# noiseinspacechannel/NIS-SAR-AMTIGMTI-Video

Measured on AMD Instinct MI355X. Metric: focused SAR frames/sec (CSA focus, complex64), higher is better.
Workload: dtype c64 (phase arguments f64)

## Files before the change

### nis-sar-amtigmti-video_amd/csrc/api_csa.hip

```cpp
#include "api_ctx.h"
#include "csa_kernels.h"
#include "general.h"

#include <cmath>
#include <cstdlib>
#include <string>
#include <vector>

using namespace sarx;

struct sarx_plan {
    sarx_ctx* ctx = nullptr;
    int n_az = 0, n_rg = 0;
    unsigned flags = 0;
    sarx_radar_params p{};
    int az_s = 0;
    int az_w = 32;
    int az_w_alone = 0;
    int az_impl = 1;
    int az_wpb = 4;
    int look = 0;
    float* look_slot = nullptr;
    float* look_part = nullptr;
    const float2* ati_s1 = nullptr; const float* ati_thr = nullptr; float ati_frac = 0.f; double ati_cal = 0.0;
    float *ati_phase = nullptr, *ati_m1 = nullptr, *ati_dm = nullptr; int ati_keep_image = 0;
    double2* ati_part = nullptr; int ati_nparts = 0;
    int ati_w = 32;
    float* max_slot = nullptr;
    bool az_nt = false;
    int slab_tiles = 0;
    double2 *c1 = nullptr, *c2 = nullptr, *c3 = nullptr;
    float2* buf_b = nullptr;
    float2* buf_a = nullptr;
    float2 *h_in = nullptr, *h_out = nullptr;
    static constexpr int PIPE = 2;
    float2 *pipe_in[PIPE] = {}, *pipe_out[PIPE] = {};
    int pipe_dl[PIPE] = {-1, -1};
    void* pipe_host[PIPE] = {};
    int pipe_next = 0;
    uint64_t bytes = 0;
    int mark_start = -1, mark_stop = -1;
    unsigned long long* stamp = nullptr;
    GeneralCsa* gen = nullptr;
// ... 186 lines not shown
                                                        "products need whole waves (sarx_ati_dpca_dev otherwise)", p->n_az, p->n_rg, tpt);
    p->ati_w = w;
    const int tiles = (p->az_s == p->n_az ? 1 : p->n_az / p->az_s) * (p->n_rg / w);
    const int waves = tpt / 64;
    if (!p->ati_part) {
        hipError_t e = hipMalloc(&p->ati_part, ((size_t)tiles * waves + 128) * sizeof(double2));
        if (e != hipSuccess) return fail(c, SARX_ERR_NOMEM, "hipMalloc ATI partial sums: %s", hipGetErrorString(e));
        p->bytes += (size_t)tiles * waves * sizeof(double2);
    }
    p->ati_nparts = tiles * waves;
    p->ati_s1 = (const float2*)d_slc1; p->ati_thr = d_max; p->ati_frac = mask_frac; p->ati_cal = cal_phase;
    p->ati_phase = d_ati_phase_masked; p->ati_m1 = d_slc1_mag; p->ati_dm = d_dpca_mag; p->ati_keep_image = keep_image != 0;
    return SARX_OK;
}

int sarx_csa_plan_bytes(const sarx_plan* p, uint64_t* out) {
    if (!p || !out) return fail(p ? p->ctx : nullptr, SARX_ERR_INVALID, "NULL argument");
    *out = p->bytes;
    return SARX_OK;
}

int sarx_csa_axes(const sarx_plan* p, double* range_axis, double* cross_range_axis) {
    if (!p) return fail(nullptr, SARX_ERR_INVALID, "plan is NULL");
    const double dt = 1.0 / p->p.sample_rate_hz;
    if (range_axis)
        for (int j = 0; j < p->n_rg; ++j) range_axis[j] = C_LIGHT * (p->p.t_start_fast_s + (double)j * dt) / 2.0;
    if (cross_range_axis) {
        double mean = 0.0;
        for (int i = 0; i < p->n_az; ++i) mean += (double)i / p->p.prf_hz;
        mean /= (double)p->n_az;
// ... 46 lines not shown
    a.ati_part = p->ati_part; a.ati_keep_image = p->ati_keep_image;
}
static int ati_finish(sarx_plan* p) {
    if (!p->ati_s1) return SARX_OK;
    sarx_ctx* c = p->ctx;
    HIPCHK(c, launch_ati_finish_sums(p->ati_part, p->ati_nparts, p->ati_thr, p->ati_part + p->ati_nparts, c->ati_out3_(), c->stream));
    return SARX_OK;
}
struct AzLast { int epi, w; };
static AzLast az_last(const sarx_plan* p, bool inv, int w_plain, AzArgs& a) {
    const bool look = inv && p->look_slot;
    if (look) { a.look_part = p->look_part; a.look = p->look; }
    const bool ati = inv && p->ati_s1;
    if (inv && !ati) a.max_out = reinterpret_cast<unsigned*>(p->max_slot);
    if (ati) ati_args(p, a);
    return {inv ? (ati ? AZ_EPI_SCALE_ATI : look ? AZ_EPI_SCALE_LOOK : AZ_EPI_SCALE) : AZ_EPI_PHI1, ati ? p->ati_w : look ? p->az_w : w_plain};
}
static int az_step(sarx_plan* p, bool inv, bool step_b, int S, const void* in, void* out, int q0, int nq) {
    sarx_ctx* c = p->ctx;
    const int n = p->n_az, RA = n / S;
    AzArgs a = az_args(p, in, out);
    a.q0 = q0;
    const bool alone = !(c->range_cus > 0 && c->range_cus < c->cus);
    const int w_plain = (alone && p->az_w_alone) ? p->az_w_alone : p->az_w;
    const auto wave = [&](int r, int epi) { return p->az_impl && n == 16384 && az_wave_supported(r, p->n_rg, epi, p->az_wpb); };
    if (!step_b) {
        a.tw_r = c->tw_all + RA;
        a.in_q_stride = 1; a.in_m_stride = S; a.out_q_stride = 1; a.out_m_stride = S;
        if (wave(RA, AZ_EPI_TWIDDLE)) HIPCHK(c, launch_az_wave(inv, AZ_EPI_TWIDDLE, p->az_wpb, a, nq, c->stream));
        else HIPCHK(c, launch_az_tile(RA, w_plain, inv, AZ_EPI_TWIDDLE, a, nq, c->stream));
    } else {
// ... 135 lines not shown
    if (p->flags & SARX_FUSE_RANGE) {
        RangeArgs a = range_args(p, p->buf_b, p->buf_b);
        a.stamp = p->stamp;
        HIPCHK(c, run_range(p, RG_FUSED, a));
    } else if (range_wp_supported(p->n_rg) && (c->range_impl == 0 || c->range_impl == 4)) {
        RangeArgs a = range_args(p, p->buf_b, p->buf_b);
        HIPCHK(c, launch_range_wp(RG_FFT_PHI2, a, c->cus, c->stream));
        HIPCHK(c, launch_range_wp(RG_IFFT_PHI3, a, c->cus, c->stream));
    } else {
        RangeArgs a = range_args(p, p->buf_b, p->buf_b);
        HIPCHK(c, run_range(p, RG_FFT_PHI2, a));
        HIPCHK(c, run_range(p, RG_IFFT_PHI3, a));
    }
    if (p->mark_stop >= 0) { HIPCHK(c, hipEventRecord(c->ev[p->mark_stop], c->stream)); c->ev_set[p->mark_stop] = true; }
    float2* last = rg_major ? p->buf_a : (float2*)d_image;
    if (p->az_s == p->n_az) {
        if ((rc = az_pass(p, true, p->buf_b, nullptr, last)) != SARX_OK) return rc;
    } else {
        if ((rc = az_pass(p, true, p->buf_b, p->buf_b, last)) != SARX_OK) return rc;
    }
    if ((rc = look_finish(p)) != SARX_OK) return rc;
    if ((rc = ati_finish(p)) != SARX_OK) return rc;
    if (rg_major) HIPCHK(c, launch_corner_turn(p->buf_a, (float2*)d_image, p->n_az, p->n_rg, c->stream));
    return SARX_OK;
}


int sarx_csa_focus_host_c128(sarx_plan* p, const void* phist_host, void* image_host) {
    if (!p) return fail(nullptr, SARX_ERR_INVALID, "plan is NULL");
    sarx_ctx* c = p->ctx;
    hipSetDevice(c->device);
// ... 71 lines not shown
```

### nis-sar-amtigmti-video_amd/csrc/csa_kernels.h

```cpp
#pragma once
#include <hip/hip_runtime.h>
#include <stddef.h>
#include <stdint.h>

namespace sarx {

enum RangeMode { RG_FFT = 0, RG_IFFT = 1, RG_FFT_PHI2 = 2, RG_IFFT_PHI3 = 3, RG_FUSED = 4,
                 RG_CONV = 5 };
enum AzEpilogue { AZ_EPI_NONE = 0, AZ_EPI_TWIDDLE = 1, AZ_EPI_PHI1 = 2, AZ_EPI_SCALE = 3,
                  AZ_EPI_TWCOL = 4,
                  AZ_EPI_PROCOL = 5,
                  AZ_EPI_ROWVEC = 6,
                  AZ_EPI_TWIDDLE_PADIN = 7,
                  AZ_EPI_CROPOUT = 8,
                  AZ_EPI_TWIDDLE_ROWSIN = 9,
                  AZ_EPI_SCALE_ROWSOUT = 10,
                  AZ_EPI_CROPOUT_PHI1 = 11,
                  AZ_EPI_CROPOUT_MAG = 12,
                  AZ_EPI_SCALE_LOOK = 13,
                  AZ_EPI_SCALE_ATI = 14 };

struct RangeArgs {
    const float2* in;
    float2* out;
    const float2* tw;
    const double2* c2;
    const double2* c3;
    double df;
    double dt;
    double t_start;
    double t0;
    float inv_n;
    int n_az;
    const float2* mulvec;
// ... 172 lines not shown
```

### nis-sar-amtigmti-video_amd/csrc/csa_kernels.hip

```cpp
#include <type_traits>
#include "csa_kernels.h"
#include "fft_core.hpp"
#include "phase.hpp"
#include "ati_pixel.hpp"

namespace sarx {

template <int N> struct RangeCfg {
    using PL = Plan<N>;
    static constexpr int T = PL::T;
    static constexpr int ROWS = (T >= 256) ? 1 : 256 / T;
    static constexpr int THREADS = T * ROWS;
    static constexpr int LDS_PER_ROW = LdsSize<N, 1>::value;
    static constexpr size_t LDS_BYTES = (size_t)ROWS * LDS_PER_ROW * sizeof(cf);
};

template <int N, int MODE>
__global__ __launch_bounds__(RangeCfg<N>::THREADS, (N == 4096 && MODE == RG_CONV) ? 4 : 1) void range_pass_kernel(RangeArgs a) {
    using CFG = RangeCfg<N>;
    using PL = Plan<N>;
    constexpr int P = PL::P, T = PL::T;
    extern __shared__ __attribute__((aligned(16))) char smem_raw[];
    cf* lds = reinterpret_cast<cf*>(smem_raw);

// ... 168 lines not shown
    static constexpr int TPC = PL::T;
    static constexpr int THREADS = TPC * W;
    static constexpr size_t LDS_BYTES = (PL::nstages > 1) ? (size_t)LdsSize<R, W>::value * sizeof(cf) : 0;
};

typedef float nt_v2f __attribute__((ext_vector_type(2)));
__device__ __forceinline__ cf ld_stream(const cf* p, bool nt) {
    if (nt) { const nt_v2f v = __builtin_nontemporal_load(reinterpret_cast<const nt_v2f*>(p)); return make_float2(v.x, v.y); }
    return *p;
}
__device__ __forceinline__ void st_stream(cf* p, cf x, bool nt) {
    if (nt) __builtin_nontemporal_store(nt_v2f{x.x, x.y}, reinterpret_cast<nt_v2f*>(p));
    else *p = x;
}

template <int R, int W, bool INV, int EPI>
__global__ __launch_bounds__((AzCfg<R, W>::THREADS)) void az_tile_kernel(AzArgs a) {
    using PL = Plan<R>;
    using E = Edge<R, false>;
    constexpr int P = PL::P;
    extern __shared__ __attribute__((aligned(16))) char smem_raw[];
    cf* lds = reinterpret_cast<cf*>(smem_raw);

    const int c = threadIdx.x % W;
    const int t = threadIdx.x / W;
    const int col = blockIdx.x * W + c;
    const int q = blockIdx.y + a.q0;
    const size_t in_base = (size_t)q * a.in_q_stride;
    const size_t out_base = (size_t)q * a.out_q_stride;

    cf v[P];
    constexpr int R0 = E::R_first;
#pragma unroll
    for (int b = 0; b < P / R0; ++b)
#pragma unroll
        for (int r = 0; r < R0; ++r) {
            const int mi = E::in_index(t, b, r);
            const size_t rowi = in_base + (size_t)mi * a.in_m_stride;
            cf x;
            if constexpr (EPI == AZ_EPI_TWIDDLE_PADIN) {
                x = make_float2(0.f, 0.f);
                if (rowi < (size_t)a.io_rows && col < a.io_cols) {
                    size_t srow = rowi + (size_t)a.io_shift_in;
                    if (srow >= (size_t)a.io_rows) srow -= (size_t)a.io_rows;
                    x = a.in[srow * a.io_ld + col];
                }
            } else if constexpr (EPI == AZ_EPI_TWIDDLE_ROWSIN) {
// ... 17 lines not shown
                for (int r = 0; r < R0; ++r) {
                    const size_t rowi = in_base + (size_t)E::in_index(t, b, r) * a.in_m_stride;
                    if (rowi >= (size_t)a.io_rows) continue;
                    cf& x = v[b * R0 + r];
                    if (a.hamming_inv > 0.f) {
                        size_t srow = rowi + (size_t)a.io_shift_in;
                        if (srow >= (size_t)a.io_rows) srow -= (size_t)a.io_rows;
                        const float w = fmaf(-0.46f, __builtin_amdgcn_cosf((float)srow * a.hamming_inv), 0.54f);
                        x.x *= w; x.y *= w;
                    } else {
                        x = cmul(x, a.rowvec[rowi]);
                    }
                }
        }
    }
    float ati_thr = 0.f;
    double ati_re = 0.0, ati_im = 0.0;
    if constexpr (EPI == AZ_EPI_SCALE_ATI) {
        __shared__ float s_m[AzCfg<R, W>::THREADS / 64 > 0 ? AzCfg<R, W>::THREADS / 64 : 1];
        float m = 0.f;
        for (unsigned k = threadIdx.x; k < MAX_SHARDS; k += AzCfg<R, W>::THREADS) m = fmaxf(m, a.ati_thr[32 * k]);
        for (int off = 32; off > 0; off >>= 1) m = fmaxf(m, __shfl_xor(m, off, 64));
        if ((threadIdx.x & 63) == 0) s_m[threadIdx.x >> 6] = m;
        __syncthreads();
        m = s_m[0];
        for (int k = 1; k < AzCfg<R, W>::THREADS / 64; ++k) m = fmaxf(m, s_m[k]);
        ati_thr = m * a.ati_frac;
    }
    cf s1v[EPI == AZ_EPI_SCALE_ATI ? P : 1];
    if constexpr (EPI == AZ_EPI_SCALE_ATI) {
        constexpr int RLp = E::R_last;
#pragma unroll
        for (int b = 0; b < P / RLp; ++b)
#pragma unroll
            for (int r = 0; r < RLp; ++r)
                s1v[b * RLp + r] = a.ati_s1[(out_base + (size_t)E::out_index(t, b, r) * a.out_m_stride) * a.n_rg + col];
    }
    stockham_run<R, W, INV, false, 0, false, (R == 128)>(v, t, c, lds, a.tw_r);
    constexpr int RL = E::R_last;
    float vmax = 0.f;
#pragma unroll
    for (int b = 0; b < P / RL; ++b)
#pragma unroll
        for (int r = 0; r < RL; ++r) {
            const int m = E::out_index(t, b, r);
            const size_t rowo = out_base + (size_t)m * a.out_m_stride;
            cf x = v[b * RL + r];
            if constexpr (EPI == AZ_EPI_TWIDDLE || EPI == AZ_EPI_TWIDDLE_PADIN || EPI == AZ_EPI_TWIDDLE_ROWSIN) {
#if SARX_HW_TWIDDLE
                const float rev = (float)(q * m) * a.scale;
                x = cmul(x, cis_frac(INV ? rev : -rev));
#else
                cf w = a.tw_n[(size_t)q * m];
                if (INV) w = cconj(w);
                x = cmul(x, w);
#endif
            } else if constexpr (EPI == AZ_EPI_PHI1) {
                x = cmul(x, phi1(col, a.c1[rowo], a.dt, a.t_start));
            } else if constexpr (EPI == AZ_EPI_SCALE_ATI) {
                x.x *= a.scale; x.y *= a.scale;
                const size_t o = rowo * a.n_rg + col;
                Pix px;
                ati_pixel<false>(s1v[b * RL + r], x, a.ati_cc, a.ati_cs, px);
                a.ati_phase[o] = px.m1 > ati_thr ? px.phase : 0.f;
                a.ati_m1[o] = px.m1;
                a.ati_dm[o] = px.dm;
                ati_re += px.sre; ati_im += px.sim;
                if (!a.ati_keep_image) continue;
            } else if constexpr (EPI == AZ_EPI_SCALE_LOOK) {
                x.x *= a.scale; x.y *= a.scale;
                if (a.max_out) vmax = fmaxf(vmax, hypotf(x.x, x.y));
                float pw = fmaf(x.x, x.x, x.y * x.y);
                auto dpp_add = [&](auto ctrl) {
                    pw += __int_as_float(__builtin_amdgcn_update_dpp(0, __float_as_int(pw), decltype(ctrl)::value, 0xF, 0xF, false));
                };
                if (a.look > 1) dpp_add(std::integral_constant<int, 0xB1>{});
                if (a.look > 2) dpp_add(std::integral_constant<int, 0x4E>{});
                if (a.look > 4) dpp_add(std::integral_constant<int, 0x141>{});
                if (a.look > 8) dpp_add(std::integral_constant<int, 0x140>{});
                for (int off = 16; off < a.look; off <<= 1) pw += __shfl_xor(pw, off, 64);
                if ((c & (a.look - 1)) == 0) a.look_part[rowo * (size_t)(a.n_rg / a.look) + col / a.look] = pw;
            } else if constexpr (EPI == AZ_EPI_SCALE || EPI == AZ_EPI_PROCOL) {
                if constexpr (EPI == AZ_EPI_PROCOL) {
                    if (a.valid_len && m * a.n_rg + col >= a.valid_len) continue;
                }
                x.x *= a.scale; x.y *= a.scale;
                if constexpr (EPI == AZ_EPI_SCALE) { if (a.max_out) vmax = fmaxf(vmax, hypotf(x.x, x.y)); }
            } else if constexpr (EPI == AZ_EPI_SCALE_ROWSOUT) {
                if (rowo >= (size_t)a.io_rows) continue;
                x.x *= a.scale; x.y *= a.scale;
            } else if constexpr (EPI == AZ_EPI_ROWVEC) {
                x = cmul(x, a.rowvec[rowo]);
            } else if constexpr (EPI == AZ_EPI_CROPOUT || EPI == AZ_EPI_CROPOUT_PHI1 || EPI == AZ_EPI_CROPOUT_MAG) {
                if (rowo < (size_t)a.io_rows && col < a.io_cols) {
                    x.x *= a.scale; x.y *= a.scale;
                    if (a.rowvec) x = cmul(x, a.rowvec[rowo]);
                    if constexpr (EPI == AZ_EPI_CROPOUT_PHI1) x = cmul(x, phi1(col, a.c1[rowo], a.dt, a.t_start));
                    size_t drow = rowo + (size_t)a.io_shift_out;
                    if (drow >= (size_t)a.io_rows) drow -= (size_t)a.io_rows;
                    if constexpr (EPI == AZ_EPI_CROPOUT_MAG) a.out_mag[drow * a.io_ld + col] = hypotf(x.x, x.y);
                    else a.out[drow * a.io_ld + col] = x;
                }
                continue;
            } else if constexpr (EPI == AZ_EPI_TWCOL) {
                const float rev = (float)(col * m) * a.tw_scale;
                x = cmul(x, cis_frac(INV ? rev : -rev));
            }
            st_stream(a.out + rowo * a.n_rg + col, x, a.nt);
        }
    if constexpr (EPI == AZ_EPI_SCALE_ATI) {
        for (int off = 32; off > 0; off >>= 1) { ati_re += __shfl_xor(ati_re, off, 64); ati_im += __shfl_xor(ati_im, off, 64); }
        if ((threadIdx.x & 63) == 0)
            a.ati_part[((size_t)blockIdx.y * gridDim.x + blockIdx.x) * (AzCfg<R, W>::THREADS / 64) + (threadIdx.x >> 6)] = make_double2(ati_re, ati_im);
    }
    if constexpr (EPI == AZ_EPI_SCALE || EPI == AZ_EPI_SCALE_LOOK) {
        if (a.max_out) {
            for (int off = 32; off > 0; off >>= 1) vmax = fmaxf(vmax, __shfl_xor(vmax, off, 64));
            if ((threadIdx.x & 63) == 0)
                atomicMax(a.max_out + 32u * ((blockIdx.x * 7u + blockIdx.y * 13u + (threadIdx.x >> 6)) & (MAX_SHARDS - 1u)), __float_as_uint(vmax));
        }
    }
}

template <int R, int W, bool INV, int EPI> static hipError_t launch_az_one(const AzArgs& a, int nq, hipStream_t st) {
    using CFG = AzCfg<R, W>;
    dim3 grid(a.n_rg / W, nq);
    hipLaunchKernelGGL((az_tile_kernel<R, W, INV, EPI>), grid, dim3(CFG::THREADS), CFG::LDS_BYTES, st, a);
    return hipGetLastError();
}
template <int R, int W> static hipError_t launch_az_rw(bool inv, int epi, const AzArgs& a, int nq, hipStream_t st) {
// ... 4 lines not shown
            case AZ_EPI_PHI1: return launch_az_one<R, W, false, AZ_EPI_PHI1>(a, nq, st);
            case AZ_EPI_TWCOL: return launch_az_one<R, W, false, AZ_EPI_TWCOL>(a, nq, st);
            case AZ_EPI_ROWVEC: return launch_az_one<R, W, false, AZ_EPI_ROWVEC>(a, nq, st);
            case AZ_EPI_TWIDDLE_PADIN: return launch_az_one<R, W, false, AZ_EPI_TWIDDLE_PADIN>(a, nq, st);
            case AZ_EPI_TWIDDLE_ROWSIN: return launch_az_one<R, W, false, AZ_EPI_TWIDDLE_ROWSIN>(a, nq, st);
            case AZ_EPI_CROPOUT:
                if constexpr (R >= 16 && W == 32) return launch_az_one<R, W, false, AZ_EPI_CROPOUT>(a, nq, st); else return hipErrorInvalidValue;
        }
    } else {
        switch (epi) {
            case AZ_EPI_NONE: return launch_az_one<R, W, true, AZ_EPI_NONE>(a, nq, st);
            case AZ_EPI_TWIDDLE: return launch_az_one<R, W, true, AZ_EPI_TWIDDLE>(a, nq, st);
            case AZ_EPI_SCALE: return launch_az_one<R, W, true, AZ_EPI_SCALE>(a, nq, st);
            case AZ_EPI_SCALE_LOOK: return launch_az_one<R, W, true, AZ_EPI_SCALE_LOOK>(a, nq, st);
            case AZ_EPI_SCALE_ATI: if constexpr (AzCfg<R, W>::THREADS % 64 == 0) return launch_az_one<R, W, true, AZ_EPI_SCALE_ATI>(a, nq, st); else return hipErrorInvalidValue;
            case AZ_EPI_PROCOL: return launch_az_one<R, W, true, AZ_EPI_PROCOL>(a, nq, st);
            case AZ_EPI_CROPOUT: return launch_az_one<R, W, true, AZ_EPI_CROPOUT>(a, nq, st);
            case AZ_EPI_SCALE_ROWSOUT: return launch_az_one<R, W, true, AZ_EPI_SCALE_ROWSOUT>(a, nq, st);
            case AZ_EPI_CROPOUT_PHI1: return launch_az_one<R, W, true, AZ_EPI_CROPOUT_PHI1>(a, nq, st);
            case AZ_EPI_CROPOUT_MAG: return launch_az_one<R, W, true, AZ_EPI_CROPOUT_MAG>(a, nq, st);
        }
    }
    return hipErrorInvalidValue;
}
template <int R> static hipError_t launch_az_r(int w, bool inv, int epi, const AzArgs& a, int nq, hipStream_t st) {
    switch (w) {
        case 16: return launch_az_rw<R, 16>(inv, epi, a, nq, st);
        case 32: return launch_az_rw<R, 32>(inv, epi, a, nq, st);
        case 64: return launch_az_rw<R, 64>(inv, epi, a, nq, st);
    }
// ... 76 lines not shown
```

### nis-sar-amtigmti-video_amd/sarx/_ffi.py

```python
from __future__ import annotations

import ctypes as C
import os

_HERE = os.path.dirname(os.path.abspath(__file__))
LIB_PATH = os.environ.get("SARX_LIB") or os.path.join(_HERE, "libsarx.so")

MAX_SLOT_BYTES = 32768
COMM_ID_BYTES = 128
OUT_AZ_MAJOR, OUT_RG_MAJOR, FUSE_RANGE = 0, 1, 2
PASS_AZ_FFT_PHI1, PASS_RG_FFT_PHI2, PASS_RG_IFFT_PHI3, PASS_AZ_IFFT, PASS_RG_FUSED_23 = 1, 2, 3, 4, 23
PASS_TEST_RG_FFT, PASS_TEST_RG_IFFT = 100, 101
PASS_RG_FFT_PHI2_PERM, PASS_RG_IFFT_PHI3_PERM = 12, 13


class SarxError(RuntimeError):

    def __init__(self, code, msg):
        super().__init__(f"libsarx error {code}: {msg}")
        self.code = code


class RadarParams(C.Structure):
    _fields_ = [(n, C.c_double) for n in (
        "wavelength_m", "pulse_width_s", "chirp_rate_hz_s", "sample_rate_hz", "prf_hz",
        "platform_speed_mps", "range_ref_m", "t_start_fast_s")]

# ... 339 lines not shown
    _fields_ = [("v_los", C.c_double), ("v_coarse", C.c_double), ("cost", C.c_double), ("cost_next", C.c_double), ("phase", C.c_double * 3),
                ("k", C.c_int32), ("status", C.c_uint32)]


_MULTI_ARGS = [_vp, _P(_vp), _vp, _vp, _vp, _d, _vp, _d, _P(TdbpMultiParams), _vp, _vp]
TDBP_MULTI_SIGNATURES = {
    "sarx_tdbp_multi_check": (_i, [_i, _P(TdbpMultiParams)]),
    "sarx_tdbp_multi_dev": (_i, _MULTI_ARGS),
    "sarx_tdbp_multi_host": (_i, _MULTI_ARGS),
    "sarx_tdbp_multi_route": (_i, [_vp, _P(_i)]),
    "sarx_tdbp_multi_scratch": (_i, [_vp, _P(_u64), _P(_u64)]),
    "sarx_tdbp_multi_resolve_check": (_i, [_P(TdbpMultiResolveParams)]),
    "sarx_tdbp_multi_resolve_dev": (_i, [_vp, _P(TdbpMultiResolveParams), _vp, _i, _i, _vp, _vp]),
}

_lib = None


def load():
    global _lib
    if _lib is not None:
        return _lib
    if not os.path.exists(LIB_PATH):
        raise SarxError(-3, f"{LIB_PATH} not built; run `python -c 'import __graft_entry__ as g; g.build()'` "
                            "or `make -C nis-sar-amtigmti-video_amd/csrc` (hipcc, gfx950). There is no CPU fallback.")
    lib = C.CDLL(LIB_PATH)
    for name, (res, args) in list(SIGNATURES.items()) + list(GMTI_SIGNATURES.items()) + list(REFOCUS_SIGNATURES.items()) + \
            list(BALANCE_SIGNATURES.items()) + list(TRACK_SIGNATURES.items()) + list(COHERENCE_SIGNATURES.items()) + list(OSCFAR_SIGNATURES.items()) + \
            list(CLUSTER_SIGNATURES.items()) + list(ATIGATE_SIGNATURES.items()) + list(TDBP_SEARCH_SIGNATURES.items()) + \
            list(TDBP_PAIR_SIGNATURES.items()) + list(TDBP_PAIR_SEARCH_SIGNATURES.items()) + list(TDBP_MULTI_SIGNATURES.items()):
        fn = getattr(lib, name)
        fn.restype = res
        fn.argtypes = args
    _lib = lib
    return lib


def check(rc, ctx=None):
    if rc != 0:
        msg = load().sarx_last_error(ctx)
        raise SarxError(rc, msg.decode() if msg else "unknown")
```

### nis-sar-amtigmti-video_amd/sarx/batch.py

```python
from __future__ import annotations

import numpy as np


def shard_frames(n_frames, world_size, rank):
    if not (0 <= rank < world_size):
        raise ValueError("rank out of range")
    return list(range(rank, n_frames, world_size))


def rounds(n_frames, world_size):
    return -(-n_frames // world_size)


def stack_from_rounds(round_blocks, n_frames):
    stack = np.concatenate([np.asarray(b) for b in round_blocks], axis=0)
    return stack[:n_frames]


def normalise_stack(stack):
    g_max = float(np.max(np.abs(stack))) if stack.size else 0.0
    g_max = g_max if g_max > 0 else 1.0
    return stack / g_max, g_max

# ... 118 lines not shown


STACKS = ("multilook", "magnitude", "products", "detections")


class _Ptr:
    def __init__(self, ptr):
        self.ptr = ptr


class TwoChannelBatch:

    def __init__(self, ctx, n, n_frames, world=1, rank=0, stack="multilook", looks=16, rccl=False, host_comm=None,
                 seed_base=1000, flags=None, mask_frac=0.05, resident=True, fused_mask=True, fused_ati=True, scene="noise",
                 scene_scale=1.0, lanes=None, detect=None, refocus=None, track=None,
                 frame_dt_s=0.1, cluster=None, ati_gate=None):
        from . import _ffi, radar
        from .engine import CsaPlan
        if stack not in STACKS:
            raise ValueError(f"stack must be one of {STACKS}")
        for name, stage in (("track", track), ("cluster", cluster), ("ati_gate", ati_gate)):
            if stage is not None and stack != "detections":
                raise ValueError(f'{name} needs stack="detections"')
        if world > 1 and not rccl and host_comm is None:
            raise ValueError("world > 1 needs a transport (rccl=True or host_comm)")
        self.ctx, self.n, self.n_frames, self.world, self.rank = ctx, int(n), int(n_frames), int(world), int(rank)
        self.stack_kind, self.looks, self.rccl, self.host_comm = stack, int(looks), bool(rccl), host_comm
        self.seed_base, self.mask_frac = int(seed_base), float(mask_frac)
        px = self.n * self.n
        self.px = px
        if scene not in ("noise", "c3"):
# ... 43 lines not shown
                self.plots_offset = self.gmti_bytes + extra
                extra += clu.plots_bytes(self._cluster_cp)
            self.gate_params = ati_gate
            self._gate = (ati_gate.c_params(self.detect.max_detections), None) if ati_gate is not None else None
            self._scratch = ("reports", "gated")[:(cluster is not None) + (ati_gate is not None)]
            for k in self._scratch:
                for st in self._lane_state:
                    st[k] = ctx.alloc(self.gmti_bytes)
            self.slot_shape = ((self.gmti_bytes + extra) // 4,)
        else:
            self.detect = None
            self.cluster_params = None
            self.gate_params = None
            self.slot_shape = (n // looks, n // looks) if stack == "multilook" else (n, n) if stack == "magnitude" else (3, n, n)
        self.slot_bytes = int(np.prod(self.slot_shape)) * 4
        self.n_rounds = rounds(self.n_frames, self.world)
        self.mine = shard_frames(self.n_frames, self.world, self.rank)
        self.d_stack = ctx.alloc(self.slot_bytes * self.world * self.n_rounds)
        if track is not None:
            import dataclasses
            from . import track as trk
            self.track_params = dataclasses.replace(track, max_detections=self.detect.max_detections)
            self._track_cp = self.track_params.c_params()
            self.d_track = (ctx.alloc(trk.table_bytes(self._track_cp)), ctx.alloc(trk.workspace_bytes(self._track_cp)),
                            ctx.alloc(self.n_frames * self.detect.max_detections * 4))
        self.resident = bool(resident)
        n_buf = len(self.mine) if self.resident else self.lanes
        rows = self.n + (1 if scene == "c3" else 0)
        self._alloc = [(ctx.alloc(rows * self.n * 8), ctx.alloc(rows * self.n * 8)) for _ in range(max(n_buf, 1))]
        self.raw = [(_Ptr(a.ptr + (self.n * 8 if scene == "c3" else 0)), _Ptr(b.ptr)) for a, b in self._alloc]
        self._prepared = False

    plan = property(lambda self: self._lane_state[self._cur]["plan"])
    s1 = property(lambda self: self._lane_state[self._cur]["s1"])
    s2 = property(lambda self: self._lane_state[self._cur]["s2"])
    outs = property(lambda self: self._lane_state[self._cur]["outs"])
    masked = property(lambda self: self._lane_state[self._cur]["masked"])
    d_max = property(lambda self: self._lane_state[self._cur]["d_max"])

    def use_lane(self, lane):
        self._cur = int(lane) % self.lanes
        self.ctx.select_lane(self.lane_ids[self._cur])

    def synth_frame(self, f, slot):
        if self.scene == "noise":
            self.ctx.fill_noise(self.raw[slot][0], self.px, self.seed_base + 2 * f)
            self.ctx.fill_noise(self.raw[slot][1], self.px, self.seed_base + 2 * f + 1)
            return
        from . import radar
# ... 17 lines not shown

    def prepare(self):
        if self.resident and not self._prepared:
            for i, f in enumerate(self.mine):
                self.synth_frame(f, i)
            self.ctx.sync()
        self._prepared = True

    def focus_frame(self, bufs, slot_ptr=None):
        ctx = self.ctx
        fused = slot_ptr is not None and self.stack_kind == "multilook"
        if fused:
            self.plan.set_look_slot(self.looks, slot_ptr)
        if self.fused_mask:
            self.plan.set_max_slot(self.d_max)
        self.plan.focus_dev(bufs[0], self.s1)
        if fused:
            self.plan.set_look_slot(self.looks, None)
        if self.fused_mask:
            self.plan.set_max_slot(None)
        if self.fused_ati:
            self._slot_written = slot_ptr is not None and self.stack_kind in ("magnitude", "products")
            masked, mag, dm = self.masked, self.outs["slc1_mag"], self.outs["dpca_mag"]
            if self._slot_written and self.stack_kind == "magnitude":
                mag = _Ptr(slot_ptr)
            elif self._slot_written:
                masked, mag, dm = (_Ptr(slot_ptr + i * self.px * 4) for i in range(3))
            self.plan.set_ati(self.s1, self.d_max, self.mask_frac, 0.0, masked, mag, dm, keep_image=self.detect is not None)
            self.plan.focus_dev(bufs[1], self.s2)
            self.plan.set_ati(None)
            self._detect(dm, slot_ptr)
            return
        self.plan.focus_dev(bufs[1], self.s2)
        self._slot_written = False
        outs, masked = self.outs, self.masked
        if slot_ptr is not None and self.stack_kind == "products":
            masked = _Ptr(slot_ptr)
            outs = dict(self.outs, slc1_mag=_Ptr(slot_ptr + self.px * 4), dpca_mag=_Ptr(slot_ptr + 2 * self.px * 4))
            self._slot_written = True
        if self.fused_mask:
            outs = dict(outs, ati_phase=masked)
            ctx.ati_dpca_masked(self.s1, self.s2, self.px, 0.0, self.d_max, self.mask_frac, outs)
        else:
            ctx.ati_dpca(self.s1, self.s2, self.px, 0.0, outs, want_stats=False)
# ... 141 lines not shown
    def stack(self, frames=None):
        if frames is None:
            return self.d_stack.download(np.float32, (self.n_rounds * self.world, *self.slot_shape))[:self.n_frames]
        out = np.empty((len(frames), *self.slot_shape), dtype=np.float32)
        from ._ffi import check
        for k, f in enumerate(frames):
            check(self.ctx.lib.sarx_memcpy_d2h(self.ctx.h, out[k].ctypes.data, self.d_stack.ptr + f * self.slot_bytes,
                                               self.slot_bytes), self.ctx.h)
        return out

    def close(self):
        self.ctx.select_lane(0)
        for b in (self.d_stack, *(x for pair in self._alloc for x in pair)):
            b.release()
        for st in self._lane_state:
            for b in (st["s1"], st["s2"], st["masked"], st["d_max"], *st["outs"].values(), *(st[k] for k in ("reports", "gated") if k in st)):
                b.release()
            st["plan"].close()
        if hasattr(self, "d_gmax"):
            self.d_gmax.release()
        if self.track_params is not None:
            for b in self.d_track:
                b.release()
```

### nis-sar-amtigmti-video_amd/sarx/engine.py

```python
from __future__ import annotations

import ctypes as C
import os
import threading
import weakref

import numpy as np

from . import _ffi
from ._ffi import SarxError, check


class DeviceBuffer:

    def __init__(self, ctx, nbytes):
        self.ctx = ctx
        self.nbytes = int(nbytes)
        p = C.c_void_p()
        check(ctx.lib.sarx_malloc(ctx.h, self.nbytes, C.byref(p)), ctx.h)
        self.ptr = p.value
        ctx._live[id(self)] = self.ptr

    def release(self):
        if self.ptr is not None and self.ctx.h is not None:
# ... 472 lines not shown
        check(self.ctx.lib.sarx_csa_plan_stamp_range(self.h, pair_ptr if pair_ptr else None), self.ctx.h)

    def set_look_slot(self, looks, slot_ptr):
        check(self.ctx.lib.sarx_csa_plan_set_look_slot(self.h, int(looks), slot_ptr if slot_ptr else None), self.ctx.h)

    def set_max_slot(self, d_max):
        check(self.ctx.lib.sarx_csa_plan_set_max_slot(self.h, d_max.ptr if d_max is not None else None), self.ctx.h)

    def set_ati(self, d_slc1, d_max=None, mask_frac=0.05, cal_phase=0.0, masked=None, slc1_mag=None, dpca_mag=None, keep_image=False):
        if d_slc1 is None:
            check(self.ctx.lib.sarx_csa_plan_set_ati(self.h, None, None, 0.0, 0.0, None, None, None, 0), self.ctx.h)
            return
        check(self.ctx.lib.sarx_csa_plan_set_ati(self.h, d_slc1.ptr, d_max.ptr, float(mask_frac), float(cal_phase), masked.ptr,
                                                 slc1_mag.ptr, dpca_mag.ptr, int(bool(keep_image))), self.ctx.h)

    def focus_dev(self, d_phist, d_image):
        check(self.ctx.lib.sarx_csa_focus_dev(self.h, d_phist.ptr, d_image.ptr), self.ctx.h)

    def run_pass(self, pass_id, d_in, d_out):
        check(self.ctx.lib.sarx_csa_pass(self.h, int(pass_id), d_in.ptr, d_out.ptr), self.ctx.h)


class FocusLanes:

    def __init__(self, ctx, n_az, n_rg, *focus_args, lanes=None, flags=_ffi.FUSE_RANGE, range_cus=192):
        if lanes is None:
            lanes = 2 if int(n_az) * int(n_rg) >= 4096 * 4096 else 1
        self.ctx, self.lanes, self.range_cus = ctx, max(1, min(int(lanes), 4)), int(range_cus)
        self.plans = [CsaPlan(ctx, n_az, n_rg, *focus_args, flags=flags) for _ in range(self.lanes)]
        self.lane_ids = ctx.concurrent_lanes(self.lanes)
# ... 49 lines not shown
```

Before: 262.7.

## Skip storing first-channel image; recompute its last azimuth transform inside the ATI pass

For the fused ATI pair route, the first channel's focus stops before the final azimuth inverse transform and writes only reductions (max and multilook power), keeping the pre-transform rows. The second channel's last azimuth kernel then loads those rows, runs the Stockham FFT on them alongside its own data, and computes the ATI products in-register. The aim is to remove a full-image write and readback of the first focused image, at the cost of extra FFT work and register pressure in the ATI epilogue. A lazy property rebuilds the first image only when something asks for it.

New measurement: 254.5. -3.1%, worse.

```diff
diff --git a/include/sarx_pair.h b/include/sarx_pair.h
--- /dev/null
+++ b/include/sarx_pair.h
@@ -0,0 +1,17 @@
+#ifndef SARX_PAIR_H
+#define SARX_PAIR_H
+
+#include "sarx.h"
+
+#ifdef __cplusplus
+extern "C" {
+#endif
+
+int sarx_csa_plan_set_reduce_only(sarx_plan* plan, int on);
+int sarx_csa_plan_set_ati_pre(sarx_plan* plan, int on);
+
+#ifdef __cplusplus
+}
+#endif
+
+#endif
diff --git a/nis-sar-amtigmti-video_amd/csrc/api_csa.hip b/nis-sar-amtigmti-video_amd/csrc/api_csa.hip
--- a/nis-sar-amtigmti-video_amd/csrc/api_csa.hip
+++ b/nis-sar-amtigmti-video_amd/csrc/api_csa.hip
@@ -1,4 +1,5 @@
 #include "api_ctx.h"
+#include "../../include/sarx_pair.h"
 #include "csa_kernels.h"
 #include "general.h"
 
@@ -27,6 +28,8 @@
     double2* ati_part = nullptr; int ati_nparts = 0;
     int ati_w = 32;
     float* max_slot = nullptr;
+    bool reduce_only = false;
+    bool ati_pre = false;
     bool az_nt = false;
     int slab_tiles = 0;
     double2 *c1 = nullptr, *c2 = nullptr, *c3 = nullptr;
@@ -243,6 +246,30 @@
     return SARX_OK;
 }
 
+static const char* pair_route_refusal(const sarx_plan* p) {
+    if (p->gen) return "any-size plans keep the stored first image (sarx_csa_plan_set_ati)";
+    if ((p->flags & SARX_OUT_RG_MAJOR) || p->slab_tiles > 0) return "the default image layout without slab mode only";
+    if (p->az_impl && p->n_az == 16384 && az_wave_supported(p->n_az / p->az_s, p->n_rg, AZ_EPI_SCALE, p->az_wpb))
+        return "16384-line plans run their last azimuth step as wave-private tiles, which have no such epilogue";
+    return nullptr;
+}
+
+int sarx_csa_plan_set_reduce_only(sarx_plan* p, int on) {
+    if (!p) return fail(nullptr, SARX_ERR_INVALID, "plan is NULL");
+    if (!on) { p->reduce_only = false; return SARX_OK; }
+    if (const char* why = pair_route_refusal(p)) return fail(p->ctx, SARX_ERR_UNSUPPORTED, "reduce-only focus: %s", why);
+    p->reduce_only = true;
+    return SARX_OK;
+}
+
+int sarx_csa_plan_set_ati_pre(sarx_plan* p, int on) {
+    if (!p) return fail(nullptr, SARX_ERR_INVALID, "plan is NULL");
+    if (!on) { p->ati_pre = false; return SARX_OK; }
+    if (const char* why = pair_route_refusal(p)) return fail(p->ctx, SARX_ERR_UNSUPPORTED, "ATI products from the first channel's pre-transform rows: %s", why);
+    p->ati_pre = true;
+    return SARX_OK;
+}
+
 int sarx_csa_plan_bytes(const sarx_plan* p, uint64_t* out) {
     if (!p || !out) return fail(p ? p->ctx : nullptr, SARX_ERR_INVALID, "NULL argument");
     *out = p->bytes;
@@ -319,7 +346,10 @@
     const bool ati = inv && p->ati_s1;
     if (inv && !ati) a.max_out = reinterpret_cast<unsigned*>(p->max_slot);
     if (ati) ati_args(p, a);
-    return {inv ? (ati ? AZ_EPI_SCALE_ATI : look ? AZ_EPI_SCALE_LOOK : AZ_EPI_SCALE) : AZ_EPI_PHI1, ati ? p->ati_w : look ? p->az_w : w_plain};
+    const bool red = inv && !ati && p->reduce_only;
+    const int epi = !inv ? AZ_EPI_PHI1 : ati ? (p->ati_pre ? AZ_EPI_SCALE_ATI_PAIR : AZ_EPI_SCALE_ATI)
+                                       : look ? (red ? AZ_EPI_SCALE_LOOK_RED : AZ_EPI_SCALE_LOOK) : (red ? AZ_EPI_SCALE_RED : AZ_EPI_SCALE);
+    return {epi, ati ? p->ati_w : look ? p->az_w : w_plain};
 }
 static int az_step(sarx_plan* p, bool inv, bool step_b, int S, const void* in, void* out, int q0, int nq) {
     sarx_ctx* c = p->ctx;
@@ -485,7 +515,16 @@
     }
     if (p->mark_stop >= 0) { HIPCHK(c, hipEventRecord(c->ev[p->mark_stop], c->stream)); c->ev_set[p->mark_stop] = true; }
     float2* last = rg_major ? p->buf_a : (float2*)d_image;
-    if (p->az_s == p->n_az) {
+    if (p->reduce_only && !p->ati_s1) {
+        const int S = p->az_s;
+        if (S == p->n_az) {
+            HIPCHK(c, hipMemcpyAsync(d_image, p->buf_b, (size_t)p->n_az * p->n_rg * sizeof(float2), hipMemcpyDeviceToDevice, c->stream));
+            if ((rc = az_pass(p, true, d_image, nullptr, d_image)) != SARX_OK) return rc;
+        } else {
+            if ((rc = az_step(p, true, false, S, p->buf_b, d_image, 0, S)) != SARX_OK) return rc;
+            if ((rc = az_step(p, true, true, S, d_image, d_image, 0, p->n_az / S)) != SARX_OK) return rc;
+        }
+    } else if (p->az_s == p->n_az) {
         if ((rc = az_pass(p, true, p->buf_b, nullptr, last)) != SARX_OK) return rc;
     } else {
         if ((rc = az_pass(p, true, p->buf_b, p->buf_b, last)) != SARX_OK) return rc;
diff --git a/nis-sar-amtigmti-video_amd/csrc/csa_kernels.h b/nis-sar-amtigmti-video_amd/csrc/csa_kernels.h
--- a/nis-sar-amtigmti-video_amd/csrc/csa_kernels.h
+++ b/nis-sar-amtigmti-video_amd/csrc/csa_kernels.h
@@ -18,6 +18,9 @@
                   AZ_EPI_CROPOUT_PHI1 = 11,
                   AZ_EPI_CROPOUT_MAG = 12,
                   AZ_EPI_SCALE_LOOK = 13,
+                  AZ_EPI_SCALE_RED = 15,
+                  AZ_EPI_SCALE_LOOK_RED = 16,
+                  AZ_EPI_SCALE_ATI_PAIR = 17,
                   AZ_EPI_SCALE_ATI = 14 };
 
 struct RangeArgs {
diff --git a/nis-sar-amtigmti-video_amd/csrc/csa_kernels.hip b/nis-sar-amtigmti-video_amd/csrc/csa_kernels.hip
--- a/nis-sar-amtigmti-video_amd/csrc/csa_kernels.hip
+++ b/nis-sar-amtigmti-video_amd/csrc/csa_kernels.hip
@@ -206,11 +206,28 @@
     else *p = x;
 }
 
+template <int THREADS> __device__ __forceinline__ float ati_threshold(const AzArgs& a) {
+    __shared__ float s_m[THREADS / 64 > 0 ? THREADS / 64 : 1];
+    float m = 0.f;
+    for (unsigned k = threadIdx.x; k < MAX_SHARDS; k += THREADS) m = fmaxf(m, a.ati_thr[32 * k]);
+    for (int off = 32; off > 0; off >>= 1) m = fmaxf(m, __shfl_xor(m, off, 64));
+    if ((threadIdx.x & 63) == 0) s_m[threadIdx.x >> 6] = m;
+    __syncthreads();
+    m = s_m[0];
+    for (int k = 1; k < THREADS / 64; ++k) m = fmaxf(m, s_m[k]);
+    return m * a.ati_frac;
+}
+
 template <int R, int W, bool INV, int EPI>
 __global__ __launch_bounds__((AzCfg<R, W>::THREADS)) void az_tile_kernel(AzArgs a) {
     using PL = Plan<R>;
     using E = Edge<R, false>;
     constexpr int P = PL::P;
+    constexpr bool PAIR = EPI == AZ_EPI_SCALE_ATI_PAIR;
+    constexpr bool ATI = EPI == AZ_EPI_SCALE_ATI || PAIR;
+    constexpr bool RED = EPI == AZ_EPI_SCALE_RED || EPI == AZ_EPI_SCALE_LOOK_RED;
+    constexpr bool LOOK = EPI == AZ_EPI_SCALE_LOOK || EPI == AZ_EPI_SCALE_LOOK_RED;
+    constexpr bool PLAIN = EPI == AZ_EPI_SCALE || EPI == AZ_EPI_SCALE_RED;
     extern __shared__ __attribute__((aligned(16))) char smem_raw[];
     cf* lds = reinterpret_cast<cf*>(smem_raw);
 
@@ -223,6 +240,17 @@
 
     cf v[P];
     constexpr int R0 = E::R_first;
+    float ati_thr = 0.f;
+    double ati_re = 0.0, ati_im = 0.0;
+    cf s1v[ATI ? P : 1];
+    if constexpr (PAIR) {
+        ati_thr = ati_threshold<AzCfg<R, W>::THREADS>(a);
+#pragma unroll
+        for (int b = 0; b < P / R0; ++b)
+#pragma unroll
+            for (int r = 0; r < R0; ++r)
+                s1v[b * R0 + r] = ld_stream(a.ati_s1 + (in_base + (size_t)E::in_index(t, b, r) * a.in_m_stride) * a.n_rg + col, a.nt);
+    }
 #pragma unroll
     for (int b = 0; b < P / R0; ++b)
 #pragma unroll
@@ -270,20 +298,7 @@
                 }
         }
     }
-    float ati_thr = 0.f;
-    double ati_re = 0.0, ati_im = 0.0;
-    if constexpr (EPI == AZ_EPI_SCALE_ATI) {
-        __shared__ float s_m[AzCfg<R, W>::THREADS / 64 > 0 ? AzCfg<R, W>::THREADS / 64 : 1];
-        float m = 0.f;
-        for (unsigned k = threadIdx.x; k < MAX_SHARDS; k += AzCfg<R, W>::THREADS) m = fmaxf(m, a.ati_thr[32 * k]);
-        for (int off = 32; off > 0; off >>= 1) m = fmaxf(m, __shfl_xor(m, off, 64));
-        if ((threadIdx.x & 63) == 0) s_m[threadIdx.x >> 6] = m;
-        __syncthreads();
-        m = s_m[0];
-        for (int k = 1; k < AzCfg<R, W>::THREADS / 64; ++k) m = fmaxf(m, s_m[k]);
-        ati_thr = m * a.ati_frac;
-    }
-    cf s1v[EPI == AZ_EPI_SCALE_ATI ? P : 1];
+    if constexpr (EPI == AZ_EPI_SCALE_ATI) ati_thr = ati_threshold<AzCfg<R, W>::THREADS>(a);
     if constexpr (EPI == AZ_EPI_SCALE_ATI) {
         constexpr int RLp = E::R_last;
 #pragma unroll
@@ -291,10 +306,17 @@
 #pragma unroll
             for (int r = 0; r < RLp; ++r)
                 s1v[b * RLp + r] = a.ati_s1[(out_base + (size_t)E::out_index(t, b, r) * a.out_m_stride) * a.n_rg + col];
+    }
+    if constexpr (PAIR) {
+        stockham_run<R, W, INV, false, 0, false, (R == 128)>(s1v, t, c, lds, a.tw_r);
+#pragma unroll
+        for (int i = 0; i < P; ++i) { s1v[i].x *= a.scale; s1v[i].y *= a.scale; }
+        if constexpr (PL::nstages > 1) __syncthreads();
     }
     stockham_run<R, W, INV, false, 0, false, (R == 128)>(v, t, c, lds, a.tw_r);
     constexpr int RL = E::R_last;
     float vmax = 0.f;
+    float pwv[EPI == AZ_EPI_SCALE_LOOK_RED ? P : 1];
 #pragma unroll
     for (int b = 0; b < P / RL; ++b)
 #pragma unroll
@@ -313,7 +335,7 @@
 #endif
             } else if constexpr (EPI == AZ_EPI_PHI1) {
                 x = cmul(x, phi1(col, a.c1[rowo], a.dt, a.t_start));
-            } else if constexpr (EPI == AZ_EPI_SCALE_ATI) {
+            } else if constexpr (ATI) {
                 x.x *= a.scale; x.y *= a.scale;
                 const size_t o = rowo * a.n_rg + col;
                 Pix px;
@@ -323,7 +345,7 @@
                 a.ati_dm[o] = px.dm;
                 ati_re += px.sre; ati_im += px.sim;
                 if (!a.ati_keep_image) continue;
-            } else if constexpr (EPI == AZ_EPI_SCALE_LOOK) {
+            } else if constexpr (LOOK) {
                 x.x *= a.scale; x.y *= a.scale;
                 if (a.max_out) vmax = fmaxf(vmax, hypotf(x.x, x.y));
                 float pw = fmaf(x.x, x.x, x.y * x.y);
@@ -335,13 +357,14 @@
                 if (a.look > 4) dpp_add(std::integral_constant<int, 0x141>{});
                 if (a.look > 8) dpp_add(std::integral_constant<int, 0x140>{});
                 for (int off = 16; off < a.look; off <<= 1) pw += __shfl_xor(pw, off, 64);
-                if ((c & (a.look - 1)) == 0) a.look_part[rowo * (size_t)(a.n_rg / a.look) + col / a.look] = pw;
-            } else if constexpr (EPI == AZ_EPI_SCALE || EPI == AZ_EPI_PROCOL) {
+                if constexpr (RED) pwv[b * RL + r] = pw;
+                else if ((c & (a.look - 1)) == 0) a.look_part[rowo * (size_t)(a.n_rg / a.look) + col / a.look] = pw;
+            } else if constexpr (PLAIN || EPI == AZ_EPI_PROCOL) {
                 if constexpr (EPI == AZ_EPI_PROCOL) {
                     if (a.valid_len && m * a.n_rg + col >= a.valid_len) continue;
                 }
                 x.x *= a.scale; x.y *= a.scale;
-                if constexpr (EPI == AZ_EPI_SCALE) { if (a.max_out) vmax = fmaxf(vmax, hypotf(x.x, x.y)); }
+                if constexpr (PLAIN) { if (a.max_out) vmax = fmaxf(vmax, hypotf(x.x, x.y)); }
             } else if constexpr (EPI == AZ_EPI_SCALE_ROWSOUT) {
                 if (rowo >= (size_t)a.io_rows) continue;
                 x.x *= a.scale; x.y *= a.scale;
@@ -362,14 +385,29 @@
                 const float rev = (float)(col * m) * a.tw_scale;
                 x = cmul(x, cis_frac(INV ? rev : -rev));
             }
+            if constexpr (RED) continue;
             st_stream(a.out + rowo * a.n_rg + col, x, a.nt);
         }
-    if constexpr (EPI == AZ_EPI_SCALE_ATI) {
+    if constexpr (EPI == AZ_EPI_SCALE_LOOK_RED) {
+        const int j = c & (a.look - 1);
+        const size_t ld = (size_t)(a.n_rg / a.look);
+        const int cg = col / a.look;
+#pragma unroll
+        for (int k = 0; k < P; ++k) {
+            if (k * a.look >= P) break;
+            const int e = j + k * a.look;
+            float sel = pwv[0];
+#pragma unroll
+            for (int i = 1; i < P; ++i) sel = (i == e) ? pwv[i] : sel;
+            if (e < P) a.look_part[(out_base + (size_t)E::out_index(t, e / RL, e % RL) * a.out_m_stride) * ld + cg] = sel;
+        }
+    }
+    if constexpr (ATI) {
         for (int off = 32; off > 0; off >>= 1) { ati_re += __shfl_xor(ati_re, off, 64); ati_im += __shfl_xor(ati_im, off, 64); }
         if ((threadIdx.x & 63) == 0)
             a.ati_part[((size_t)blockIdx.y * gridDim.x + blockIdx.x) * (AzCfg<R, W>::THREADS / 64) + (threadIdx.x >> 6)] = make_double2(ati_re, ati_im);
     }
-    if constexpr (EPI == AZ_EPI_SCALE || EPI == AZ_EPI_SCALE_LOOK) {
+    if constexpr (PLAIN || LOOK) {
         if (a.max_out) {
             for (int off = 32; off > 0; off >>= 1) vmax = fmaxf(vmax, __shfl_xor(vmax, off, 64));
             if ((threadIdx.x & 63) == 0)
@@ -404,6 +442,9 @@
             case AZ_EPI_SCALE: return launch_az_one<R, W, true, AZ_EPI_SCALE>(a, nq, st);
             case AZ_EPI_SCALE_LOOK: return launch_az_one<R, W, true, AZ_EPI_SCALE_LOOK>(a, nq, st);
             case AZ_EPI_SCALE_ATI: if constexpr (AzCfg<R, W>::THREADS % 64 == 0) return launch_az_one<R, W, true, AZ_EPI_SCALE_ATI>(a, nq, st); else return hipErrorInvalidValue;
+            case AZ_EPI_SCALE_ATI_PAIR: if constexpr (AzCfg<R, W>::THREADS % 64 == 0) return launch_az_one<R, W, true, AZ_EPI_SCALE_ATI_PAIR>(a, nq, st); else return hipErrorInvalidValue;
+            case AZ_EPI_SCALE_RED: return launch_az_one<R, W, true, AZ_EPI_SCALE_RED>(a, nq, st);
+            case AZ_EPI_SCALE_LOOK_RED: return launch_az_one<R, W, true, AZ_EPI_SCALE_LOOK_RED>(a, nq, st);
             case AZ_EPI_PROCOL: return launch_az_one<R, W, true, AZ_EPI_PROCOL>(a, nq, st);
             case AZ_EPI_CROPOUT: return launch_az_one<R, W, true, AZ_EPI_CROPOUT>(a, nq, st);
             case AZ_EPI_SCALE_ROWSOUT: return launch_az_one<R, W, true, AZ_EPI_SCALE_ROWSOUT>(a, nq, st);
diff --git a/nis-sar-amtigmti-video_amd/sarx/_ffi.py b/nis-sar-amtigmti-video_amd/sarx/_ffi.py
--- a/nis-sar-amtigmti-video_amd/sarx/_ffi.py
+++ b/nis-sar-amtigmti-video_amd/sarx/_ffi.py
@@ -11,6 +11,7 @@
 OUT_AZ_MAJOR, OUT_RG_MAJOR, FUSE_RANGE = 0, 1, 2
 PASS_AZ_FFT_PHI1, PASS_RG_FFT_PHI2, PASS_RG_IFFT_PHI3, PASS_AZ_IFFT, PASS_RG_FUSED_23 = 1, 2, 3, 4, 23
 PASS_TEST_RG_FFT, PASS_TEST_RG_IFFT = 100, 101
+PASS_TEST_AZ_INV_A, PASS_TEST_AZ_INV_B = 112, 113
 PASS_RG_FFT_PHI2_PERM, PASS_RG_IFFT_PHI3_PERM = 12, 13
 
 
@@ -380,6 +381,11 @@
     "sarx_tdbp_multi_resolve_dev": (_i, [_vp, _P(TdbpMultiResolveParams), _vp, _i, _i, _vp, _vp]),
 }
 
+PAIR_SIGNATURES = {
+    "sarx_csa_plan_set_reduce_only": (_i, [_vp, _i]),
+    "sarx_csa_plan_set_ati_pre": (_i, [_vp, _i]),
+}
+
 _lib = None
 
 
@@ -394,7 +400,8 @@
     for name, (res, args) in list(SIGNATURES.items()) + list(GMTI_SIGNATURES.items()) + list(REFOCUS_SIGNATURES.items()) + \
             list(BALANCE_SIGNATURES.items()) + list(TRACK_SIGNATURES.items()) + list(COHERENCE_SIGNATURES.items()) + list(OSCFAR_SIGNATURES.items()) + \
             list(CLUSTER_SIGNATURES.items()) + list(ATIGATE_SIGNATURES.items()) + list(TDBP_SEARCH_SIGNATURES.items()) + \
-            list(TDBP_PAIR_SIGNATURES.items()) + list(TDBP_PAIR_SEARCH_SIGNATURES.items()) + list(TDBP_MULTI_SIGNATURES.items()):
+            list(TDBP_PAIR_SIGNATURES.items()) + list(TDBP_PAIR_SEARCH_SIGNATURES.items()) + list(TDBP_MULTI_SIGNATURES.items()) + \
+            list(PAIR_SIGNATURES.items()):
         fn = getattr(lib, name)
         fn.restype = res
         fn.argtypes = args
diff --git a/nis-sar-amtigmti-video_amd/sarx/batch.py b/nis-sar-amtigmti-video_amd/sarx/batch.py
--- a/nis-sar-amtigmti-video_amd/sarx/batch.py
+++ b/nis-sar-amtigmti-video_amd/sarx/batch.py
@@ -156,7 +156,7 @@
     def __init__(self, ctx, n, n_frames, world=1, rank=0, stack="multilook", looks=16, rccl=False, host_comm=None,
                  seed_base=1000, flags=None, mask_frac=0.05, resident=True, fused_mask=True, fused_ati=True, scene="noise",
                  scene_scale=1.0, lanes=None, detect=None, refocus=None, track=None,
-                 frame_dt_s=0.1, cluster=None, ati_gate=None):
+                 frame_dt_s=0.1, cluster=None, ati_gate=None, pair_route=True):
         from . import _ffi, radar
         from .engine import CsaPlan
         if stack not in STACKS:
@@ -230,6 +230,16 @@
             self.gate_params = None
             self.slot_shape = (n // looks, n // looks) if stack == "multilook" else (n, n) if stack == "magnitude" else (3, n, n)
         self.slot_bytes = int(np.prod(self.slot_shape)) * 4
+        self.pair_route = bool(pair_route) and self.fused_ati and self.detect is None
+        if self.pair_route:
+            try:
+                for st in self._lane_state:
+                    st["plan"].set_reduce_only(True)
+                    st["plan"].set_reduce_only(False)
+            except _ffi.SarxError as e:
+                if e.code != -2:
+                    raise
+                self.pair_route = False
         self.n_rounds = rounds(self.n_frames, self.world)
         self.mine = shard_frames(self.n_frames, self.world, self.rank)
         self.d_stack = ctx.alloc(self.slot_bytes * self.world * self.n_rounds)
@@ -248,7 +258,20 @@
         self._prepared = False
 
     plan = property(lambda self: self._lane_state[self._cur]["plan"])
-    s1 = property(lambda self: self._lane_state[self._cur]["s1"])
+    @property
+    def s1(self):
+        st = self._lane_state[self._cur]
+        if not st.get("s1_rows"):
+            return st["s1"]
+        if st.get("s1_img") is None:
+            st["s1_img"] = self.ctx.alloc(self.px * 8)
+        if not st["s1_img_valid"]:
+            from . import _ffi
+            self.ctx.select_lane(self.lane_ids[self._cur])
+            st["plan"].run_pass(_ffi.PASS_AZ_IFFT if self.n <= 128 else _ffi.PASS_TEST_AZ_INV_B, st["s1"], st["s1_img"])
+            st["s1_img_valid"] = True
+        return st["s1_img"]
+
     s2 = property(lambda self: self._lane_state[self._cur]["s2"])
     outs = property(lambda self: self._lane_state[self._cur]["outs"])
     masked = property(lambda self: self._lane_state[self._cur]["masked"])
@@ -296,7 +319,14 @@
             self.plan.set_look_slot(self.looks, slot_ptr)
         if self.fused_mask:
             self.plan.set_max_slot(self.d_max)
-        self.plan.focus_dev(bufs[0], self.s1)
+        st = self._lane_state[self._cur]
+        s1 = st["s1"]
+        st["s1_rows"], st["s1_img_valid"] = self.pair_route, False
+        if self.pair_route:
+            self.plan.set_reduce_only(True)
+        self.plan.focus_dev(bufs[0], s1)
+        if self.pair_route:
+            self.plan.set_reduce_only(False)
         if fused:
             self.plan.set_look_slot(self.looks, None)
         if self.fused_mask:
@@ -308,8 +338,12 @@
                 mag = _Ptr(slot_ptr)
             elif self._slot_written:
                 masked, mag, dm = (_Ptr(slot_ptr + i * self.px * 4) for i in range(3))
-            self.plan.set_ati(self.s1, self.d_max, self.mask_frac, 0.0, masked, mag, dm, keep_image=self.detect is not None)
+            self.plan.set_ati(s1, self.d_max, self.mask_frac, 0.0, masked, mag, dm, keep_image=self.detect is not None)
+            if self.pair_route:
+                self.plan.set_ati_pre(True)
             self.plan.focus_dev(bufs[1], self.s2)
+            if self.pair_route:
+                self.plan.set_ati_pre(False)
             self.plan.set_ati(None)
             self._detect(dm, slot_ptr)
             return
@@ -481,7 +515,8 @@
         for b in (self.d_stack, *(x for pair in self._alloc for x in pair)):
             b.release()
         for st in self._lane_state:
-            for b in (st["s1"], st["s2"], st["masked"], st["d_max"], *st["outs"].values(), *(st[k] for k in ("reports", "gated") if k in st)):
+            for b in (st["s1"], st["s2"], st["masked"], st["d_max"], *st["outs"].values(),
+                      *(st[k] for k in ("reports", "gated", "s1_img") if st.get(k) is not None)):
                 b.release()
             st["plan"].close()
         if hasattr(self, "d_gmax"):
diff --git a/nis-sar-amtigmti-video_amd/sarx/engine.py b/nis-sar-amtigmti-video_amd/sarx/engine.py
--- a/nis-sar-amtigmti-video_amd/sarx/engine.py
+++ b/nis-sar-amtigmti-video_amd/sarx/engine.py
@@ -510,6 +510,12 @@
         check(self.ctx.lib.sarx_csa_plan_set_ati(self.h, d_slc1.ptr, d_max.ptr, float(mask_frac), float(cal_phase), masked.ptr,
                                                  slc1_mag.ptr, dpca_mag.ptr, int(bool(keep_image))), self.ctx.h)
 
+    def set_reduce_only(self, on):
+        check(self.ctx.lib.sarx_csa_plan_set_reduce_only(self.h, int(bool(on))), self.ctx.h)
+
+    def set_ati_pre(self, on):
+        check(self.ctx.lib.sarx_csa_plan_set_ati_pre(self.h, int(bool(on))), self.ctx.h)
+
     def focus_dev(self, d_phist, d_image):
         check(self.ctx.lib.sarx_csa_focus_dev(self.h, d_phist.ptr, d_image.ptr), self.ctx.h)
 
```
